# achraf-15/neural_image_compression

Measured on AMD Instinct MI355X. Metric: images/sec (256x256 RGB, batch 32) fwd+bwd, higher is better.
Workload: dtype f32; 1 GPU; cfg2: JointAutoregressiveHierarchical(M=192,K=1) fwd+rd_loss(lambda=0.01)+bwd+Adam, 32x3x256x256 per GPU, fp32; global_batch=32, parallelism=dp1, step=eager (autograd)

## Files before the change

include/lic.h:

```cpp
#ifndef LIC_H
#define LIC_H

#include <stddef.h>
#include <stdint.h>

#ifdef __cplusplus
extern "C" {
#endif

#define LIC_ABI_VERSION 4

typedef void* lic_stream_t;

enum lic_status {
  LIC_OK = 0,
  LIC_ERR_INVALID = -1,
  LIC_ERR_UNSUPPORTED = -2,
  LIC_ERR_LAUNCH = -3,
  LIC_ERR_WORKSPACE = -4
};

enum lic_epilogue {
  LIC_EPI_NONE = 0,
  LIC_EPI_LEAKY = 1,
// ... 413 lines not shown
} lic_adam_job;
int64_t lic_adam_plan(lic_adam_job* jobs, int32_t njobs);
int lic_adam_run(const lic_adam_job* jobs_device, int32_t njobs, int64_t total_blocks, const float* const* grads_host,
                 double lr, double beta1, double beta2, double eps, double weight_decay, double bias_correction1,
                 double bias_correction2, lic_stream_t stream);

int lic_grad_norm_partial(const lic_adam_job* jobs_device, int32_t njobs, int64_t total_blocks,
                          const float* const* grads_host, double* partials, lic_stream_t stream);
int lic_grad_norm_finish(const double* partials, int64_t nparts, double max_norm, int32_t count_skip, float* clip_state,
                         lic_stream_t stream);
int lic_adam_run_scaled(const lic_adam_job* jobs_device, int32_t njobs, int64_t total_blocks,
                        const float* const* grads_host, double lr, double beta1, double beta2, double eps,
                        double weight_decay, double bias_correction1, double bias_correction2, const float* clip_state,
                        int32_t skip_nonfinite, lic_stream_t stream);

int lic_adam_run_ema(const lic_adam_job* jobs_device, int32_t njobs, int64_t total_blocks,
                     const float* const* grads_host, double lr, double beta1, double beta2, double eps,
                     double weight_decay, double bias_correction1, double bias_correction2, float* const* ema_device,
                     double ema_weight, const float* clip_state, int32_t skip_nonfinite, lic_stream_t stream);
int lic_swap_run(const lic_adam_job* jobs_device, int32_t njobs, int64_t total_blocks, float* const* ema_device,
                 lic_stream_t stream);

enum { LIC_REDUCE_SLABS = 0, LIC_REDUCE_COLUMNS = 1 };
enum { LIC_REDUCE_EPI_NONE = 0, LIC_REDUCE_EPI_REPARAM = 1 };
#define LIC_REDUCE_MAX_JOBS 32
typedef struct lic_reduce_job {
  const float* src;
  float* dst;
  const float* param;
  int64_t sm, smr, sn, snr, stap;
  int32_t kind, epilogue;
  int32_t splitk, ntaps, Cm, Cn, Mvalid, Nvalid, mdiv, ndiv;
  float scale, bound;
  int32_t block0, nblocks;
} lic_reduce_job;
int lic_wgrad_bf16_partial(const lic_wgrad_desc* d, void* workspace, size_t workspace_bytes, lic_reduce_job* job,
                           lic_stream_t stream);
int lic_colsum_bf16_partial(const void* in, int64_t ld, int64_t P, int32_t C, float scale, float* out, void* workspace,
                            size_t workspace_bytes, lic_reduce_job* job, lic_stream_t stream);
int lic_colsum2_bf16_partial(const void* in_a, const void* in_b, int64_t ld, int64_t P, int32_t C, float scale,
                             float* out_a, float* out_b, void* workspace, size_t workspace_bytes, lic_reduce_job* jobs2,
                             lic_stream_t stream);
int lic_leaky_bwd_colsum_bf16(const void* y, const void* dy, void* dx, int64_t P, int32_t C, float slope, float* out,
                              void* workspace, size_t workspace_bytes, lic_reduce_job* job, lic_stream_t stream);
int lic_reduce_batch(const lic_reduce_job* jobs, int32_t njobs, lic_stream_t stream);

int lic_head_convt_bf16_supported(int32_t Cin, int32_t Cout, int32_t kh, int32_t kw, int32_t stride, int32_t pad,
                                  int32_t out_pad);
int lic_head_convt_bf16(const void* x, const void* w_packed, const float* bias, float* out, int32_t B, int32_t Hi,
                        int32_t Wi, int32_t Cin, lic_stream_t stream);
int lic_stem_conv_bf16(const float* x, const void* w_packed, const float* bias, void* y, int32_t B, int32_t H, int32_t W,
                       int32_t Cout, lic_stream_t stream);

typedef struct lic_plan lic_plan;
int lic_plan_create(void* hip_graph, lic_plan** out);
int lic_plan_info(const lic_plan* plan, int64_t* info);
int lic_plan_replay(lic_plan* plan, lic_stream_t main, const lic_stream_t* sides, int32_t n_sides);
int lic_plan_tune(lic_plan* plan, lic_stream_t main, const lic_stream_t* sides, int32_t n_sides, double* result);
int lic_plan_dag(const lic_plan* plan, int64_t cap_ops, int64_t cap_edges, int64_t* sizes, int32_t* pred_ptr,
                 int32_t* pred_idx, int32_t* kind, int32_t* flags, double* us);
int lic_plan_commands(lic_plan* plan, int32_t n_sides, int64_t cap, int64_t* n_cmds, int32_t* cmds);
int lic_plan_sched_host(int64_t n_ops, const int32_t* pred_ptr, const int32_t* pred_idx, const double* us,
                        const int32_t* flags, int32_t mode, int32_t ns, double wide_min_us, int32_t n_sides,
                        int64_t cap, int64_t* n_cmds, int32_t* cmds, int64_t* info);
void lic_plan_destroy(lic_plan* plan);
const char* lic_plan_last_error(void);

int lic_version(void);
int lic_last_hip_error(void);
const char* lic_arch(void);

#ifdef __cplusplus
}
#endif
#endif
```

neural_image_compression_amd/_lib.py:

```python
from __future__ import annotations

import ctypes as C
import os

_HERE = os.path.dirname(os.path.abspath(__file__))
LIB_PATH = os.path.join(_HERE, "liblic_hip.so")

EPI_NONE, EPI_LEAKY, EPI_MUL_LEAKY_MASK, EPI_GDN, EPI_IGDN, EPI_GDN_BWD, EPI_IGDN_BWD, EPI_CONV_GDN, EPI_CONV_IGDN = range(9)
FE_NPARAM = 43

_vp, _i32, _i64, _f32, _sz = C.c_void_p, C.c_int32, C.c_int64, C.c_float, C.c_size_t


class IgemmDesc(C.Structure):
    _fields_ = [("in_", _vp), ("w", _vp), ("bias", _vp), ("out", _vp), ("out2", _vp), ("aux", _vp),
                ("aux2", _vp), ("aux3", _vp), ("res", _vp),
                ("in_ld", _i64), ("out_ld", _i64), ("out2_ld", _i64), ("aux_ld", _i64),
                ("aux2_ld", _i64), ("aux3_ld", _i64), ("res_ld", _i64),
                ("B", _i32), ("Hi", _i32), ("Wi", _i32), ("Cin", _i32),
                ("Ho", _i32), ("Wo", _i32), ("Cout", _i32),
                ("kh", _i32), ("kw", _i32), ("stride", _i32), ("pad", _i32),
                ("transposed", _i32), ("prologue", _i32), ("epilogue", _i32),
                ("tap_mask", C.c_uint32), ("slope", _f32), ("workspace", _vp), ("workspace_bytes", _sz),
                ("out3", _vp), ("out3_ld", _i64),
# ... 171 lines not shown
    "lic_gdn_fwd": (C.c_int, [_vp, _vp, _vp, _vp, _vp, _vp, _i64, _i32, _i32, _vp]),
    "lic_gdn_bwd_partial_rows": (_i64, [_i64]),
    "lic_gdn_bwd": (C.c_int, [_vp, _vp, _vp, _vp, _vp, _vp, _vp, _vp, _i64, _i32, _i32, _vp]),
    "lic_factorized_cdf_tables": (C.c_int, [_vp, _i32, _i32, _i32, _vp, _vp]),
    "lic_gmm_cdf_tables": (C.c_int, [_vp, _i64, _i32, _i32, _i32, _vp, _vp, _vp]),
    "lic_rans_decode_step": (C.c_int, [_vp] * 8 + [_i32] * 4 + [_vp, _vp, _i64, _vp]),
    "lic_rans_encode_pick": (C.c_int, [_vp] * 4 + [_i32, _i64, _i32, _i32] + [_vp] * 4),
    "lic_rans_encode": (C.c_int, [_vp] * 3 + [_i64, _i32, _i64, _vp, _i64, _vp, _vp, _vp]),
    "lic_rans_decode_step_groups": (C.c_int, [_vp] * 8 + [_i32] * 5 + [_vp, _vp, _i64, _vp]),
    "lic_rans_encode_groups": (C.c_int, [_vp] * 3 + [_i64, _i32, _i32, _i64, _vp, _i64, _vp, _i64, _vp, _vp]),
    "lic_rans_encode_pick_ragged": (C.c_int, [_vp] * 3 + [_i64, _vp, _i32, _vp, _vp, _i32, _i32] + [_vp] * 4),
    "lic_rans_encode_ragged": (C.c_int, [_vp] * 3 + [_i64, _vp, _vp, _i32, _i32, _i64, _i32, _vp, _i64, _vp, _i64,
                                         _vp, _vp]),
    "lic_ctx_gather": (C.c_int, [_vp] + [_i64] * 4 + [_i32] * 4 + [_vp, _i32, _i32, _vp, _i64, _vp, _vp, _i32, _vp, _i64,
                                 _i32, _vp]),
    "lic_ctx_gather_ragged": (C.c_int, [_vp, _i64, _i64, _vp, _i32, _i32, _vp, _i32, _vp, _vp, _i64, _vp, _vp, _i64, _i32,
                                        _vp, _i64, _i32, _vp]),
    "lic_rans_decode_step_ragged": (C.c_int, [_vp] * 9 + [_i32, _i32, _i64, _i32, _i32, _vp, _vp, _vp, _vp, _i64, _vp]),
    "lic_ctx_gather_layers": (C.c_int, [_vp] + [_i64] * 4 + [_i32] * 3 + [_vp, _i32, _i32, _vp, _i64, _vp, _i32,
                                        C.POINTER(CtxLayer), _i32, _i32, _vp]),
    "lic_rans_decode_step_layers": (C.c_int, [_vp] * 6 + [C.POINTER(RansLayer)] + [_i32] * 5 + [_vp, _vp, _i64, _i64,
                                                                                                 _vp]),
    "lic_ctx_gather_layers_ragged": (C.c_int, [_vp, _i64, _i64, _vp, _i32, _vp, _i32, _vp, _vp, _i64, _vp, _i64, _i32,
                                               C.POINTER(CtxLayer), _i32, _i32, _vp]),
    "lic_rans_decode_step_layers_ragged": (C.c_int, [_vp] * 6 + [C.POINTER(RansLayer), _i32, _vp, _i32, _i32, _i64,
                                                                 _i32, _vp, _vp, _vp, _vp, _i64, _i64, _vp]),
    "lic_rans_z_pick": (C.c_int, [_vp, _i32, _i32, _i32, _vp, _i64, _vp, _vp, _vp, _vp]),
    "lic_rans_z_decode_path": (C.c_int, [_i32, _i32]),
    "lic_rans_z_decode": (C.c_int, [_vp] * 7 + [_i32] * 5 + [_vp, _vp, _vp, _i64, _i32, _vp]),
    "lic_msssim_workspace_bytes": (_sz, [_i32, _i32, _i32, _i32]),
    "lic_msssim": (C.c_int, [_vp, _vp, _i32, _i32, _i32, _i32, _i64, _i64, _i64, _i64, _f32, _vp, _vp, _vp, _sz,
                             _vp]),
    "lic_msssim_bwd_workspace_bytes": (_sz, [_i32, _i32, _i32, _i32]),
    "lic_msssim_bwd": (C.c_int, [_vp, _vp, _i32, _i32, _i32, _i32, _i64, _i64, _i64, _i64, _f32, _vp, _vp, _sz, _vp,
                                 _vp, _vp, _sz, _vp]),
    "lic_u8_to_f32": (C.c_int, [_vp, _vp, _i64, _vp]),
    "lic_window_u8_to_f32": (C.c_int, [_vp, _vp, _i32, _i32, _i32, _i32, _i32, _vp, _vp]),
    "lic_window_f32": (C.c_int, [_vp, _i64, _i64, _i64, _i64] + [_i32] * 9 + [_vp, _vp]),
    "lic_resample_u8_to_f32": (C.c_int, [_vp, _vp, _i32, _i32, _i32, _i32, _vp, _vp]),
    "lic_tensor_stats_workspace_bytes": (_sz, []),
    "lic_tensor_stats": (C.c_int, [_vp, _i64, _i32, _f32, _f32, _vp, _vp, _vp, _sz, _vp]),
    "lic_prep_plan": (_i64, [C.POINTER(PrepJob), _i32]),
    "lic_prep_run": (C.c_int, [_vp, _i32, _i64, _vp]),
    "lic_adam_plan": (_i64, [C.POINTER(AdamJob), _i32]),
    "lic_adam_run": (C.c_int, [_vp, _i32, _i64, _vp] + [C.c_double] * 7 + [_vp]),
    "lic_grad_norm_partial": (C.c_int, [_vp, _i32, _i64, _vp, _vp, _vp]),
    "lic_grad_norm_finish": (C.c_int, [_vp, _i64, C.c_double, _i32, _vp, _vp]),
    "lic_adam_run_scaled": (C.c_int, [_vp, _i32, _i64, _vp] + [C.c_double] * 7 + [_vp, _i32, _vp]),
    "lic_adam_run_ema": (C.c_int, [_vp, _i32, _i64, _vp] + [C.c_double] * 7 + [_vp, C.c_double, _vp, _i32, _vp]),
    "lic_swap_run": (C.c_int, [_vp, _i32, _i64, _vp, _vp]),
    "lic_head_convt_bf16_supported": (C.c_int, [_i32] * 7),
    "lic_head_convt_bf16": (C.c_int, [_vp, _vp, _vp, _vp, _i32, _i32, _i32, _i32, _vp]),
    "lic_stem_conv_bf16": (C.c_int, [_vp, _vp, _vp, _vp, _i32, _i32, _i32, _i32, _vp]),
    "lic_plan_create": (C.c_int, [_vp, C.POINTER(C.c_void_p)]),
    "lic_plan_info": (C.c_int, [_vp, C.POINTER(C.c_int64)]),
    "lic_plan_replay": (C.c_int, [_vp, _vp, C.POINTER(C.c_void_p), _i32]),
    "lic_plan_tune": (C.c_int, [_vp, _vp, C.POINTER(C.c_void_p), _i32, C.POINTER(C.c_double)]),
    "lic_plan_dag": (C.c_int, [_vp, _i64, _i64, C.POINTER(C.c_int64), _vp, _vp, _vp, _vp, _vp]),
    "lic_plan_commands": (C.c_int, [_vp, _i32, _i64, C.POINTER(C.c_int64), _vp]),
    "lic_plan_sched_host": (C.c_int, [_i64, _vp, _vp, _vp, _vp, _i32, _i32, C.c_double, _i32, _i64,
                                      C.POINTER(C.c_int64), _vp, _vp]),
    "lic_plan_destroy": (None, [_vp]),
    "lic_plan_last_error": (C.c_char_p, []),
    "lic_version": (C.c_int, []),
    "lic_last_hip_error": (C.c_int, []),
    "lic_arch": (C.c_char_p, []),
}

_lib = None


class LicError(RuntimeError):
    pass


def load():
    global _lib
    if _lib is None:
        if not os.path.exists(LIB_PATH):
            raise LicError(
                f"{LIB_PATH} not found: the HIP extension is not built. Run "
                "`python -c 'import __graft_entry__ as g; g.build()'` (or make -C "
                "neural_image_compression_amd/csrc). There is no CPU fallback.")
        lib = C.CDLL(LIB_PATH)
        for name, (res, args) in SIGNATURES.items():
            fn = getattr(lib, name)
            fn.restype = res
            fn.argtypes = args
        _lib = lib
    return _lib


_STATUS = {-1: "LIC_ERR_INVALID", -2: "LIC_ERR_UNSUPPORTED", -3: "LIC_ERR_LAUNCH", -4: "LIC_ERR_WORKSPACE"}


def check(rc: int, what: str):
    if rc != 0:
        extra = f" (hipError {load().lic_last_hip_error()})" if rc == -3 else ""
        raise LicError(f"{what} failed: {_STATUS.get(rc, rc)}{extra}")
```

neural_image_compression_amd/functional.py:

```python
from __future__ import annotations

import ctypes as C
from typing import Optional, Tuple

import torch

from . import _lib as L
from .reductions import can_defer, defer, flush_point, flush_reductions

PEDESTAL = float(2.0 ** -36)
LIKELIHOOD_BOUND = 1e-9

PROFILE = None
PROFILE_MIN_FLOP = 0.0
FORCE_IGEMM = None
FORCE_WGRAD = None
KERNEL_TRACE = None
GRAD_VIEWS = {}
PREPARED = {}
AUX_STREAM = None
PLAN_RECORDING = False


_raw_stream = getattr(torch._C, "_cuda_getCurrentRawStream", None)


def _stream():
    if _raw_stream is not None:
        return C.c_void_p(_raw_stream(torch.cuda.current_device()))
    return C.c_void_p(torch.cuda.current_stream().cuda_stream)


def _ptr(t: Optional[torch.Tensor]):
    return None if t is None else C.c_void_p(t.data_ptr())


def _require_cuda(*ts):
    for t in ts:
        if t is not None and not t.is_cuda:
            raise L.LicError("neural_image_compression_amd runs on MI355X only: got a non-CUDA tensor "
                             "(there is no CPU fallback; the CPU oracle lives in oracle/ for tests)")
        if t is not None and t.device.index != torch.cuda.current_device():
            raise L.LicError(f"tensor on cuda:{t.device.index} but the current device is cuda:"
                             f"{torch.cuda.current_device()}: call torch.cuda.set_device(...) first (one process per GPU)")
        if t is not None and t.dtype != torch.float32:
            raise L.LicError(f"fp32 tensors expected, got {t.dtype}")


def _nhwc(t: torch.Tensor) -> torch.Tensor:
    return t.permute(0, 2, 3, 1).contiguous()


def _nchw_view(t_nhwc: torch.Tensor) -> torch.Tensor:
    return t_nhwc.permute(0, 3, 1, 2)


def _permute3(src, dst, n, s, d):
    L.check(L.load().lic_permute3(_ptr(src), _ptr(dst), n[0], n[1], n[2], s[0], s[1], s[2], d[0], d[1],
                                  d[2], _stream()), "lic_permute3")


def _pack(src: torch.Tensor, taps: int, K: int, N: int, s_tap: int, s_k: int, s_n: int) -> torch.Tensor:
    lib = L.load()
    out = torch.empty((lib.lic_packed_weight_floats(taps, K, N),), device=src.device, dtype=torch.float32)
    L.check(lib.lic_pack_weight(_ptr(src), _ptr(out), taps, K, N, s_tap, s_k, s_n, _stream()),
            "lic_pack_weight")
    return out


def _pack_dense(m: torch.Tensor) -> torch.Tensor:
    K, N = m.shape
    return _pack(m, 1, K, N, 0, N, 1)

# ... 410 lines not shown
                                          ctx.needs_input_grad[1], has_bias and ctx.needs_input_grad[2])
        return dx, dw, db, None, None, None, None


class _ImageConvGDNFn(torch.autograd.Function):

    @staticmethod
    def forward(ctx, x, weight, bias, beta, gamma, stride, pad, inverse, beta_bound, gamma_bound, pedestal, keep=True):
        _require_cuda(x, weight, bias, beta, gamma)
        xh = _nhwc(x)
        B = xh.shape[0]
        Cout = weight.shape[0]
        col, wp, Ho, Wo, Kp = _image_conv_columns(xh, weight, stride, pad)
        P = B * Ho * Wo
        beta_e, gT = _gdn_operands(beta, gamma, beta_bound, gamma_bound, pedestal)
        y = torch.empty((B, Ho, Wo, Cout), device=x.device, dtype=torch.float32)
        conv_out = torch.empty_like(y) if keep else None
        norm = torch.empty_like(y) if keep else None
        _igemm(col, wp, y, B=1, Hi=1, Wi=P, Cin=Kp, Ho=1, Wo=P, Cout=Cout, kh=1, kw=1, stride=1,
               pad=0, transposed=False, bias=bias, epilogue=L.EPI_CONV_IGDN if inverse else L.EPI_CONV_GDN,
               out2=norm, out3=conv_out, aux=gT, aux2=beta_e)
        ctx.save_for_backward(col, weight, conv_out, norm, beta, gamma)
        ctx.cfg = (stride, pad, tuple(xh.shape), inverse, beta_bound, gamma_bound, bias is not None, pedestal)
        return _nchw_view(y)

    @staticmethod
    def backward(ctx, gy):
        col, weight, conv_out, norm, beta, gamma = ctx.saved_tensors
        stride, pad, in_shape, inverse, beta_bound, gamma_bound, has_bias, pedestal = ctx.cfg
        need = ctx.needs_input_grad
        g_conv, dbeta, dgamma = _gdn_backward(conv_out, norm, beta, gamma, _nhwc(gy), inverse,
                                              beta_bound, gamma_bound, pedestal, True, need[3], need[4])
        dx, dw, db = _image_conv_backward(col, weight, g_conv, stride, pad, in_shape, need[0], need[1],
                                          has_bias and need[2])
        return dx, dw, db, dbeta, dgamma, None, None, None, None, None, None, None


class _ImageConvTFn(torch.autograd.Function):

    @staticmethod
    def forward(ctx, x, weight, bias, stride, pad, out_pad):
        _require_cuda(x, weight, bias)
        xh = _nhwc(x)
        B, Hi, Wi, Cin = xh.shape
        _, Cout, kh, kw = weight.shape
        Ho, Wo = conv_out_size(Hi, Wi, kh, stride, pad, True, out_pad)
        taps, Kp, P = kh * kw, _kpad(kh, kw, Cout), B * Hi * Wi
        lib = L.load()
        wpk = prepared(weight, "f32.head")
        if wpk is None:
            wp = torch.zeros((Cin, Kp), device=x.device, dtype=torch.float32)
            _permute3(weight.contiguous(), wp, (Cin, Cout, taps), (Cout * taps, taps, 1), (Kp, 1, Cout))
            wpk = _pack_dense(wp)
        col = torch.empty((P, Kp), device=x.device, dtype=torch.float32)
        _igemm(xh, wpk, col, B=1, Hi=1, Wi=P, Cin=Cin, Ho=1, Wo=P, Cout=Kp, kh=1, kw=1, stride=1, pad=0,
               transposed=False)
        out = torch.empty((B, Ho, Wo, Cout), device=x.device, dtype=torch.float32)
        L.check(lib.lic_col2im(_ptr(col), _ptr(bias), _ptr(out), B, Hi, Wi, Cout, Ho, Wo, kh, kw, stride,
                               pad, Kp, _stream()), "lic_col2im")
        ctx.save_for_backward(xh, weight)
        ctx.cfg = (stride, pad, (Ho, Wo), bias is not None)
        return _nchw_view(out)

    @staticmethod
    def backward(ctx, gy):
        xh, weight = ctx.saved_tensors
        stride, pad, (Ho, Wo), has_bias = ctx.cfg
        g = _nhwc(gy)
        B, Hi, Wi, Cin = xh.shape
        _, Cout, kh, kw = weight.shape
        taps, Kp, P = kh * kw, _kpad(kh, kw, Cout), B * Hi * Wi
        lib = L.load()
        dcol = torch.empty((P, Kp), device=g.device, dtype=torch.float32)
        L.check(lib.lic_im2col(_ptr(g), _ptr(dcol), B, Ho, Wo, Cout, Hi, Wi, kh, kw, stride, pad, Kp,
                               _stream()), "lic_im2col")
        dx = dw = db = None
        if ctx.needs_input_grad[0]:
            wpk = prepared(weight, "f32.head_dx")
            if wpk is None:
                wpT = torch.zeros((Kp, Cin), device=g.device, dtype=torch.float32)
                _permute3(weight.contiguous(), wpT, (taps, Cout, Cin), (1, taps, Cout * taps),
                          (Cout * Cin, Cin, 1))
                wpk = _pack_dense(wpT)
            dxh = torch.empty_like(xh)
            _igemm(dcol, wpk, dxh, B=1, Hi=1, Wi=P, Cin=Kp, Ho=1, Wo=P, Cout=Cin, kh=1, kw=1, stride=1,
                   pad=0, transposed=False)
            dx = _nchw_view(dxh)
        if ctx.needs_input_grad[1]:
            dw = grad_like(weight)
            tmp = torch.empty((Cin, Kp), device=g.device, dtype=torch.float32)
            _wgrad(xh, dcol, tmp, B=1, Hs=1, Ws=P, Cp=Cin, Hl=1, Wl=P, Cg=Kp, kh=1, kw=1, stride=1, pad=0,
                   g_is_row=True, dst_sm=1, dst_sn=Kp, dst_stap=0)
            _permute3(tmp, dw, (Cin, taps, Cout), (Kp, Cout, 1), (Cout * taps, 1, taps))
        if has_bias and ctx.needs_input_grad[2]:
            db = _colsum(g, B * Ho * Wo, Cout)
        return dx, dw, db, None, None, None


def image_conv2d(x, weight, bias, stride, padding, leaky=False, slope=0.01):
    return _ImageConvFn.apply(x, weight, bias, stride, padding, leaky, slope)


def image_conv_transpose2d(x, weight, bias, stride, padding, output_padding):
    return _ImageConvTFn.apply(x, weight, bias, stride, padding, output_padding)


class _LeakyFn(torch.autograd.Function):
    @staticmethod
    def forward(ctx, x, slope):
        _require_cuda(x)
        xc = x.contiguous()
        y = _leaky_bwd(xc, xc, slope)
        ctx.save_for_backward(y)
        ctx.slope = slope
        return y

    @staticmethod
    def backward(ctx, gy):
        (y,) = ctx.saved_tensors
        return _leaky_bwd(y, gy.contiguous(), ctx.slope), None


def leaky_relu(x, slope=0.01):
    return _LeakyFn.apply(x, slope)


class _GDNFn(torch.autograd.Function):
    @staticmethod
    def forward(ctx, x, beta, gamma, inverse, beta_bound, gamma_bound, pedestal, res, keep=True):
        _require_cuda(x, beta, gamma, res)
        lib = L.load()
        xh = _nhwc(x)
        B, H, W, Cc = xh.shape
        beta_e, gT = _gdn_operands(beta, gamma, beta_bound, gamma_bound, pedestal)
        out = torch.empty_like(xh)
        norm = torch.empty_like(xh) if keep else None
        resh = None if res is None else _nhwc(res)
        P = B * H * W
        if lib.lic_gdn_supported(Cc):
            _trace(lambda: f"gdn_kernel<{Cc // 64}, {int(inverse)}>")
            _timed(f"gdn_kernel<{Cc // 64}, 0>", 2 * P * Cc * Cc, 4 * 3 * P * Cc,
                   lambda: L.check(lib.lic_gdn_fwd(_ptr(xh), _ptr(gT), _ptr(beta_e), _ptr(resh), _ptr(out), _ptr(norm),
                                                   P, Cc, int(inverse), _stream()), "lic_gdn_fwd"))
        else:
            _igemm(xh, gT, out, B=1, Hi=1, Wi=P, Cin=Cc, Ho=1, Wo=P, Cout=Cc, kh=1, kw=1, stride=1, pad=0,
                   transposed=False, bias=beta_e, prologue=1, epilogue=L.EPI_IGDN if inverse else L.EPI_GDN,
                   out2=norm, aux=xh, res=resh)
        ctx.save_for_backward(xh, norm, beta, gamma)
        ctx.cfg = (inverse, beta_bound, gamma_bound, res is not None, pedestal)
# ... 749 lines not shown
```

neural_image_compression_amd/csrc/lic_gemm.hip:

```cpp
#include "lic_tile_map.h"
#include <stdio.h>
#include <stdlib.h>
#include <algorithm>
#include <type_traits>

thread_local int g_lic_last_hip_error = 0;

struct IgemmParams {
  const float* in;
  const float* w;
  const float* bias;
  float* out;
  float* out2;
  const float* aux;
  const float* aux2;
  const float* aux3;
  const float* res;
  float* out3;
  long in_ld, out_ld, out2_ld, aux_ld, aux2_ld, aux3_ld, res_ld, out3_ld;
  int B, Hi, Wi, Cin, Ho, Wo, Cout;
  int kw, stride, pad, transposed, prologue, epilogue;
  float slope;
  int vec;
  int vec_out;
// ... 1175 lines not shown
          for (int b = 0; b < TN; ++b)
            acc[a][b] = __builtin_amdgcn_mfma_f32_32x32x2f32(af[a][t], bf[b][t], acc[a][b], 0, 0, 0);
    } else {
#pragma unroll
      for (int a = 0; a < TM; ++a)
        if (a < m_live) {
#pragma unroll
          for (int b = 0; b < TN; ++b)
            if (b < n_live) {
#pragma unroll
              for (int t = 0; t < 8; ++t)
                acc[a][b] = __builtin_amdgcn_mfma_f32_32x32x2f32(af[a][t], bf[b][t], acc[a][b], 0, 0, 0);
            }
        }
    }
  };

  if (nloc > 0) {
    load_chunk(c_begin);
    store_chunk(0);
    __syncthreads();
    load_chunk(c_begin + 1);
    int c = 0;
    for (; c + 1 < nloc; c += 2) {
      store_chunk(1);
      load_chunk(c_begin + c + 2);
      compute(0);
      __syncthreads();
      store_chunk(0);
      load_chunk(c_begin + c + 3);
      compute(1);
      __syncthreads();
    }
    if (c < nloc) {
      compute(0);
      __syncthreads();
    }
  }
  float* slab = p.slabs + ((long)split * p.ntaps + tap) * p.row.C * p.col.C;
#pragma unroll
  for (int a = 0; a < TM; ++a)
#pragma unroll
    for (int q = 0; q < 16; ++q) {
      const int m = m0 + wm0 + a * 32 + (q & 3) + 8 * (q >> 2) + 4 * lh;
      if (m >= p.row.C) continue;
#pragma unroll
      for (int b = 0; b < TN; ++b) {
        const int n = n0 + wn0 + b * 32 + li;
        if (n < p.col.C) slab[(long)m * p.col.C + n] = acc[a][b][q];
      }
    }
}

template <int TM, int TN, bool SQB = false, bool FULL = true>
__global__ __launch_bounds__(256, (TM * TN >= 6 ? 2 : 1)) void wgrad_glds_kernel(const WgradParams p) {
  constexpr int BMt = 64 * TM, BNt = 64 * TN, NS = TM + TN;
  constexpr int WM = BMt / 2, WN = BNt / 2;
  __shared__ __attribute__((aligned(16))) float smem[2][NS][WG_BK * 64];
  const int tid = threadIdx.x, lane = tid & 63;
  const int wave = __builtin_amdgcn_readfirstlane(tid >> 6);
  const int wm0 = (wave >> 1) * WM, wn0 = (wave & 1) * WN;
  const int li = lane & 31, lh = lane >> 5;
  const WgradTile wt = wgrad_tile(p, xcd_contiguous(blockIdx.x, gridDim.x), BMt, BNt);
  const int m0 = wt.m0, n0 = wt.n0, tap = wt.tap, split = wt.split;
  const int c_begin = wt.c_begin, c_end = wt.c_end, nloc = c_end - c_begin;

  f32x16 acc[TM][TN];
#pragma unroll
  for (int a = 0; a < TM; ++a)
#pragma unroll
    for (int b = 0; b < TN; ++b)
#pragma unroll
      for (int q = 0; q < 16; ++q) acc[a][b][q] = 0.0f;

  const int kr = tid >> 4, c16 = (tid & 15) * 4;
  constexpr unsigned WG_OOB = 0x80000000u, WG_GBIAS = 0x40000000u;
  const unsigned row_ld4 = (unsigned)p.row.ld * 4u, col_ld4 = (unsigned)p.col.ld * 4u;
  const unsigned row_lin = (unsigned)kr * row_ld4 + (unsigned)c16 * 4u;
  const unsigned col_lin = (unsigned)kr * col_ld4 + (unsigned)c16 * 4u;
  const bool row_g = p.row.gathered != 0, col_g = p.col.gathered != 0;
  const unsigned g_ld4 = row_g ? row_ld4 : col_ld4;
  const unsigned HWl = (unsigned)(p.Hl * p.Wl);
  const int tap_h = wt.r - p.pad, tap_w = wt.s - p.pad;
  bool row_live[TM], col_live[TN];
#pragma unroll
  for (int j = 0; j < TM; ++j) row_live[j] = FULL || m0 + c16 + 64 * j < p.row.C;
#pragma unroll
  for (int j = 0; j < TN; ++j) col_live[j] = FULL || n0 + c16 + 64 * j < p.col.C;
  const float* const row_base = p.row.ptr + m0;
  const float* const col_base = p.col.ptr + n0;
  auto issue = [&](int c, int buf) {
    const int cc = c < c_end ? c : c_end - 1;
    const int pk0 = cc * WG_BK;
    const int b0 = fdiv(pk0, p.dHW);
    const int rem0 = pk0 - b0 * p.Hs * p.Ws;
    const int hs0 = fdiv(rem0, p.dW), ws0 = rem0 - hs0 * p.Ws;
    const long g0 = ((long)b0 * p.Hl + (hs0 * p.stride + tap_h)) * p.Wl + (ws0 * p.stride + tap_w);
    const unsigned pk = (unsigned)pk0 + (unsigned)kr;
    const int pix = pk < (unsigned)p.Ps ? (int)pk : 0;
    const int b = fdiv(pix, p.dHW);
    const int rem = pix - b * p.Hs * p.Ws;
    const int hs = fdiv(rem, p.dW), ws = rem - hs * p.Ws;
    const int hl = hs * p.stride + tap_h, wl = ws * p.stride + tap_w;
    const bool gok = pk < (unsigned)p.Ps && (unsigned)hl < (unsigned)p.Hl && (unsigned)wl < (unsigned)p.Wl;
    const unsigned dpix = (unsigned)b * HWl + (unsigned)hl * (unsigned)p.Wl + (unsigned)wl - (unsigned)g0;
    const unsigned gokm = (unsigned)(-(int)gok);
    const unsigned g_off = ((dpix * g_ld4 + (WG_GBIAS + (unsigned)c16 * 4u)) & gokm) | (~gokm & WG_OOB);
    const long left = p.Ps - pk0;
    const unsigned lin_rec = (unsigned)(left < WG_BK ? left : WG_BK);
    auto rsrc = [&](const float* base, long ld, unsigned ld4, bool gathered) {
      const long px = gathered ? g0 : (long)pk0;
      const float* b_ = base + (px * ld - (gathered ? (long)(WG_GBIAS / 4) : 0L));
      return __builtin_amdgcn_make_buffer_rsrc(const_cast<float*>(b_), 0, gathered ? (int)WG_OOB : (int)(lin_rec * ld4),
                                               0x00020000);
    };
    const __amdgpu_buffer_rsrc_t rs_row = rsrc(row_base, p.row.ld, row_ld4, row_g);
    const __amdgpu_buffer_rsrc_t rs_col = rsrc(col_base, p.col.ld, col_ld4, col_g);
    const unsigned row_off = row_g ? g_off : row_lin, col_off = col_g ? g_off : col_lin;
#pragma unroll
    for (int j = 0; j < TM; ++j)
      __builtin_amdgcn_raw_ptr_buffer_load_lds(rs_row, (lic_lptr_t)&smem[buf][j][wave * 256], 16,
                                               (int)(row_live[j] ? row_off : WG_OOB), 256 * j, 0, 0);
#pragma unroll
    for (int j = 0; j < TN; ++j)
      __builtin_amdgcn_raw_ptr_buffer_load_lds(rs_col, (lic_lptr_t)&smem[buf][TM + j][wave * 256], 16,
                                               (int)(col_live[j] ? col_off : WG_OOB), 256 * j, 0, 0);
  };
  auto compute = [&](int buf) {
    float af[TM][8], bf[TN][8];
#pragma unroll
    for (int a = 0; a < TM; ++a) {
      const int ch = wm0 + a * 32;
#pragma unroll
      for (int t = 0; t < 8; ++t) af[a][t] = smem[buf][ch >> 6][(lh * 8 + t) * 64 + (ch & 63) + li];
    }
#pragma unroll
    for (int b = 0; b < TN; ++b) {
      const int ch = wn0 + b * 32;
#pragma unroll
      for (int t = 0; t < 8; ++t) {
        const float v = smem[buf][TM + (ch >> 6)][(lh * 8 + t) * 64 + (ch & 63) + li];
        bf[b][t] = SQB ? v * v : v;
      }
    }
#pragma unroll
    for (int t = 0; t < 8; ++t)
#pragma unroll
      for (int a = 0; a < TM; ++a)
#pragma unroll
        for (int b = 0; b < TN; ++b)
          acc[a][b] = __builtin_amdgcn_mfma_f32_32x32x2f32(af[a][t], bf[b][t], acc[a][b], 0, 0, 0);
  };

  if (nloc > 0) {
    issue(c_begin, 0);
    int c = 0;
    for (; c + 1 < nloc; c += 2) {
      __syncthreads();
      issue(c_begin + c + 1, 1);
      compute(0);
      __builtin_amdgcn_sched_barrier(0);
      __syncthreads();
      issue(c_begin + c + 2, 0);
      compute(1);
      __builtin_amdgcn_sched_barrier(0);
    }
    __syncthreads();
    if (c < nloc) compute(0);
  }
  float* slab = p.slabs + ((long)split * p.ntaps + tap) * p.row.C * p.col.C;
#pragma unroll
  for (int a = 0; a < TM; ++a)
#pragma unroll
    for (int q = 0; q < 16; ++q) {
      const int m = m0 + wm0 + a * 32 + (q & 3) + 8 * (q >> 2) + 4 * lh;
      if (!FULL && m >= p.row.C) continue;
#pragma unroll
      for (int b = 0; b < TN; ++b) {
        const int n = n0 + wn0 + b * 32 + li;
        if (FULL || n < p.col.C) slab[(long)m * p.col.C + n] = acc[a][b][q];
      }
    }
}

__global__ __launch_bounds__(256) void wgrad_reduce_kernel(const float* slabs, float* dst, int splitk,
                                                           int ntaps, int Cm, int Cn, long sm, long sn,
                                                           long stap, float scale) {
  const long total = (long)ntaps * Cm * Cn;
  for (long i = (long)blockIdx.x * 256 + threadIdx.x; i < total; i += (long)gridDim.x * 256) {
    float a8[8] = {0.f, 0.f, 0.f, 0.f, 0.f, 0.f, 0.f, 0.f};
    int z = 0;
    for (; z + 8 <= splitk; z += 8) {
#pragma unroll
      for (int k = 0; k < 8; ++k) a8[k] += slabs[(long)(z + k) * total + i];
    }
    for (; z < splitk; ++z) a8[0] += slabs[(long)z * total + i];
    const float acc = ((a8[0] + a8[1]) + (a8[2] + a8[3])) + ((a8[4] + a8[5]) + (a8[6] + a8[7]));
    const int n = (int)(i % Cn);
    const long t2 = i / Cn;
    const int m = (int)(t2 % Cm);
    const int tap = (int)(t2 / Cm);
    dst[m * sm + n * sn + tap * stap] = acc * scale;
  }
}

long lic_pick_splits(long base, long slots, long max_sk) {
  long best = 1;
  double best_eff = 0.0;
  if (max_sk > 512) max_sk = 512;
  if (max_sk < 1) max_sk = 1;
  for (long r = 1; r <= 4; ++r) {
    long sk = (r * slots) / base;
    if (sk < 1) continue;
    if (sk > max_sk) sk = max_sk;
    const long wgs = base * sk;
    const double eff = (double)wgs / ((double)((wgs + slots - 1) / slots) * (double)slots);
    if (eff > best_eff + 0.03) {
      best = sk;
      best_eff = eff;
    }
    if (eff >= 0.9 || sk == max_sk) break;
// ... 157 lines not shown
```

Measured before the change: 1496 images/s.

## Fuse RGB head transposed-conv GEMM and col2im into one direct kernel

Adds a dedicated fp32 MFMA kernel for the final 5x5 stride-2 transposed conv to 3 channels. Each tile computes the per-pixel column products into LDS with halo and immediately scatters and adds them into the output image, so the large intermediate column buffer is never written to or read back from global memory. The kernel is persistent and software-pipelines input and weight loads. It recomputes the halo columns in each tile and only covers specific channel counts, falling back to the old GEMM plus col2im path otherwise.

```diff
diff --git a/include/lic.h b/include/lic.h
--- a/include/lic.h
+++ b/include/lic.h
@@ -489,6 +489,11 @@
 int lic_stem_conv_bf16(const float* x, const void* w_packed, const float* bias, void* y, int32_t B, int32_t H, int32_t W,
                        int32_t Cout, lic_stream_t stream);
 
+int lic_head_convt_f32_supported(int32_t Cin, int32_t Cout, int32_t kh, int32_t kw, int32_t stride, int32_t pad,
+                                 int32_t out_pad);
+int lic_head_convt_f32(const float* x, const float* w_packed, const float* bias, float* out, int32_t B, int32_t Hi, int32_t Wi,
+                       int32_t Cin, int32_t grid_cap, lic_stream_t stream);
+
 typedef struct lic_plan lic_plan;
 int lic_plan_create(void* hip_graph, lic_plan** out);
 int lic_plan_info(const lic_plan* plan, int64_t* info);
diff --git a/neural_image_compression_amd/_lib.py b/neural_image_compression_amd/_lib.py
--- a/neural_image_compression_amd/_lib.py
+++ b/neural_image_compression_amd/_lib.py
@@ -247,6 +247,8 @@
     "lic_head_convt_bf16_supported": (C.c_int, [_i32] * 7),
     "lic_head_convt_bf16": (C.c_int, [_vp, _vp, _vp, _vp, _i32, _i32, _i32, _i32, _vp]),
     "lic_stem_conv_bf16": (C.c_int, [_vp, _vp, _vp, _vp, _i32, _i32, _i32, _i32, _vp]),
+    "lic_head_convt_f32_supported": (C.c_int, [_i32] * 7),
+    "lic_head_convt_f32": (C.c_int, [_vp, _vp, _vp, _vp, _i32, _i32, _i32, _i32, _i32, _vp]),
     "lic_plan_create": (C.c_int, [_vp, C.POINTER(C.c_void_p)]),
     "lic_plan_info": (C.c_int, [_vp, C.POINTER(C.c_int64)]),
     "lic_plan_replay": (C.c_int, [_vp, _vp, C.POINTER(C.c_void_p), _i32]),
diff --git a/neural_image_compression_amd/csrc/lic_rgb.hip b/neural_image_compression_amd/csrc/lic_rgb.hip
--- /dev/null
+++ b/neural_image_compression_amd/csrc/lic_rgb.hip
@@ -0,0 +1,188 @@
+#include "lic_common.h"
+
+namespace {
+
+__device__ __forceinline__ void rg_lds_barrier() { asm volatile("s_waitcnt lgkmcnt(0)\n\ts_barrier" ::: "memory"); }
+
+constexpr int HF_TH = 12, HF_TW = 16;
+constexpr int HF_HR = HF_TH + 2, HF_HC = HF_TW + 2;
+constexpr int HF_HP = HF_HR * HF_HC;
+constexpr int HF_MT = (HF_HP + 31) / 32;
+constexpr int HF_LD = 84;
+constexpr int HF_THREADS = 64 * HF_MT;
+
+struct HeadFwdParams {
+  const float* x;
+  const float* w;
+  const float* bias;
+  float* out;
+  int B, Hi, Wi, tiles_x, tiles_y;
+  long ntiles;
+};
+
+template <int NC>
+__global__ __launch_bounds__(HF_THREADS, 2) void head_convt_f32_kernel(const HeadFwdParams p) {
+  constexpr int C = 16 * NC;
+  constexpr int WTS = NC * 3 * 512;
+  __shared__ __attribute__((aligned(16))) float smem[WTS + HF_MT * 32 * HF_LD];
+  float* wts = smem;
+  float* col = smem + WTS;
+  const int tid = threadIdx.x, lane = tid & 63, li = lane & 31, lh = lane >> 5;
+  const int wave = __builtin_amdgcn_readfirstlane(tid >> 6);
+  for (int v = tid; v < WTS / 4; v += HF_THREADS) {
+    const int blk = v >> 6, c = blk / 6, r = blk - 6 * c;
+    *reinterpret_cast<f32x4*>(wts + 4 * v) = *reinterpret_cast<const f32x4*>(p.w + ((long)(c * 8 + r) * 64 + (v & 63)) * 4);
+  }
+  float bs[3] = {0.f, 0.f, 0.f};
+  if (p.bias)
+#pragma unroll
+    for (int c = 0; c < 3; ++c) bs[c] = p.bias[c];
+  const int Ho = 2 * p.Hi, Wo = 2 * p.Wi;
+  const int ntiles = (int)p.ntiles;
+  const float* wl = wts + lane * 4;
+  const int hp = 32 * wave + li;
+  const int hr = hp / HF_HC, hc = hp - hr * HF_HC;
+  auto row_of = [&](int tile) {
+    const int tx = tile % p.tiles_x, rest = tile / p.tiles_x;
+    const int ty = rest % p.tiles_y, b = rest / p.tiles_y;
+    const int iy = min(max(ty * HF_TH - 1 + hr, 0), p.Hi - 1), ix = min(max(tx * HF_TW - 1 + hc, 0), p.Wi - 1);
+    return p.x + (((long)b * p.Hi + iy) * p.Wi + ix) * C + 8 * lh;
+  };
+  f32x4 a[3][2];
+  f32x4 bw[2][3][2];
+  const float* xrow = p.x;
+  auto load_a = [&](int c) {
+    a[c % 3][0] = *reinterpret_cast<const f32x4*>(xrow + 16 * c);
+    a[c % 3][1] = *reinterpret_cast<const f32x4*>(xrow + 16 * c + 4);
+  };
+  auto load_b = [&](int c) {
+#pragma unroll
+    for (int nt = 0; nt < 3; ++nt)
+#pragma unroll
+      for (int q = 0; q < 2; ++q) bw[c & 1][nt][q] = *reinterpret_cast<const f32x4*>(wl + ((c * 3 + nt) * 2 + q) * 256);
+  };
+  int tile = blockIdx.x;
+  if (tile < ntiles) {
+    xrow = row_of(tile);
+    load_a(0);
+    load_a(1);
+  }
+  rg_lds_barrier();
+
+  for (; tile < ntiles; tile += gridDim.x) {
+    const int tx = tile % p.tiles_x, rest = tile / p.tiles_x;
+    const int ty = rest % p.tiles_y, b = rest / p.tiles_y;
+    const int y0 = ty * HF_TH, x0 = tx * HF_TW;
+    f32x16 acc[3];
+#pragma unroll
+    for (int nt = 0; nt < 3; ++nt)
+#pragma unroll
+      for (int r = 0; r < 16; ++r) acc[nt][r] = 0.0f;
+    load_b(0);
+#pragma unroll
+    for (int c = 0; c < NC; ++c) {
+      if (c + 2 < NC) load_a(c + 2);
+      if (c + 1 < NC) load_b(c + 1);
+      __builtin_amdgcn_sched_barrier(0);
+#pragma unroll
+      for (int t = 0; t < 8; ++t)
+#pragma unroll
+        for (int nt = 0; nt < 3; ++nt)
+          acc[nt] = __builtin_amdgcn_mfma_f32_32x32x2f32(a[c % 3][t >> 2][t & 3], bw[c & 1][nt][t >> 2][t & 3], acc[nt], 0, 0, 0);
+    }
+    {
+      float* dst = col + (32 * wave + 4 * lh) * HF_LD + li;
+#pragma unroll
+      for (int nt = 0; nt < 3; ++nt)
+        if (32 * nt + li < 80)
+#pragma unroll
+          for (int r = 0; r < 16; ++r) dst[((r & 3) + 8 * (r >> 2)) * HF_LD + 32 * nt] = acc[nt][r] + 0.0f;
+    }
+    if (tile + (int)gridDim.x < ntiles) {
+      xrow = row_of(tile + gridDim.x);
+      load_a(0);
+      load_a(1);
+    }
+    rg_lds_barrier();
+    for (int o = tid; o < 4 * HF_TH * HF_TW; o += HF_THREADS) {
+      const int oyl = o / (2 * HF_TW), oxl = o - oyl * (2 * HF_TW);
+      const int oy = 2 * y0 + oyl, ox = 2 * x0 + oxl;
+      if (oy >= Ho || ox >= Wo) continue;
+      const int qy = oyl >> 1, py = oyl & 1, qx = oxl >> 1, px = oxl & 1;
+      float o0 = bs[0], o1 = bs[1], o2 = bs[2];
+#pragma unroll
+      for (int aa = 0; aa < 3; ++aa) {
+        const int ky = py + 2 * aa, iy = y0 + qy + 1 - aa;
+        if (ky > 4 || iy < 0 || iy >= p.Hi) continue;
+#pragma unroll
+        for (int bb = 0; bb < 3; ++bb) {
+          const int kx = px + 2 * bb, ix = x0 + qx + 1 - bb;
+          if (kx > 4 || ix < 0 || ix >= p.Wi) continue;
+          const float* c3 = col + ((qy + 2 - aa) * HF_HC + (qx + 2 - bb)) * HF_LD + 3 * (5 * ky + kx);
+          o0 += c3[0];
+          o1 += c3[1];
+          o2 += c3[2];
+        }
+      }
+      float* dst = p.out + (((long)b * Ho + oy) * Wo + ox) * 3;
+      dst[0] = o0;
+      dst[1] = o1;
+      dst[2] = o2;
+    }
+    rg_lds_barrier();
+  }
+}
+
+bool rg_al16(const void* q) { return (reinterpret_cast<uintptr_t>(q) & 15) == 0; }
+
+template <int NC>
+int head_fwd_launch(const HeadFwdParams& p, int grid_cap, hipStream_t s) {
+  static const int slots = [] {
+    int per_cu = 0, cus = 0, devid = 0;
+    if (hipOccupancyMaxActiveBlocksPerMultiprocessor(&per_cu, (const void*)head_convt_f32_kernel<NC>, HF_THREADS, 0) != hipSuccess ||
+        per_cu < 1)
+      per_cu = 1;
+    if (hipGetDevice(&devid) != hipSuccess ||
+        hipDeviceGetAttribute(&cus, hipDeviceAttributeMultiprocessorCount, devid) != hipSuccess || cus < 1)
+      cus = 256;
+    return per_cu * cus;
+  }();
+  long grid = p.ntiles < slots ? p.ntiles : slots;
+  if (grid_cap > 0 && grid > grid_cap) grid = grid_cap;
+  hipLaunchKernelGGL((head_convt_f32_kernel<NC>), dim3((unsigned)grid), dim3(HF_THREADS), 0, s, p);
+  return lic_check_launch();
+}
+
+bool rg_geometry(int Cin, int Cout, int kh, int kw, int stride, int pad, int out_pad) {
+  return (Cin == 64 || Cin == 128 || Cin == 192) && Cout == 3 && kh == 5 && kw == 5 && stride == 2 && pad == 2 && out_pad == 1;
+}
+
+}
+
+LIC_EXPORT int lic_head_convt_f32_supported(int32_t Cin, int32_t Cout, int32_t kh, int32_t kw, int32_t stride, int32_t pad,
+                                            int32_t out_pad) {
+  return rg_geometry(Cin, Cout, kh, kw, stride, pad, out_pad) ? 1 : 0;
+}
+
+LIC_EXPORT int lic_head_convt_f32(const float* x, const float* w_packed, const float* bias, float* out, int32_t B, int32_t Hi,
+                                  int32_t Wi, int32_t Cin, int32_t grid_cap, lic_stream_t stream) {
+  if (!x || !w_packed || !out || B <= 0 || Hi <= 0 || Wi <= 0 || grid_cap < 0) return LIC_ERR_INVALID;
+  if (!(Cin == 64 || Cin == 128 || Cin == 192)) return LIC_ERR_UNSUPPORTED;
+  if (!rg_al16(x) || !rg_al16(w_packed) || (reinterpret_cast<uintptr_t>(out) & 3)) return LIC_ERR_INVALID;
+  if ((long)B * Hi * Wi * Cin > 0x7FFFFFFFFFL || (long)B * Hi * Wi >= 0x7FFFFFFFL) return LIC_ERR_UNSUPPORTED;
+  HeadFwdParams p;
+  p.x = x;
+  p.w = w_packed;
+  p.bias = bias;
+  p.out = out;
+  p.B = B;
+  p.Hi = Hi;
+  p.Wi = Wi;
+  p.tiles_x = (Wi + HF_TW - 1) / HF_TW;
+  p.tiles_y = (Hi + HF_TH - 1) / HF_TH;
+  p.ntiles = (long)B * p.tiles_x * p.tiles_y;
+  hipStream_t s = (hipStream_t)stream;
+  if (Cin == 64) return head_fwd_launch<4>(p, grid_cap, s);
+  if (Cin == 128) return head_fwd_launch<8>(p, grid_cap, s);
+  return head_fwd_launch<12>(p, grid_cap, s);
+}
diff --git a/neural_image_compression_amd/functional.py b/neural_image_compression_amd/functional.py
--- a/neural_image_compression_amd/functional.py
+++ b/neural_image_compression_amd/functional.py
@@ -19,6 +19,7 @@
 GRAD_VIEWS = {}
 PREPARED = {}
 AUX_STREAM = None
+RGB_DIRECT = True
 PLAN_RECORDING = False
 
 
@@ -535,12 +536,15 @@
             wp = torch.zeros((Cin, Kp), device=x.device, dtype=torch.float32)
             _permute3(weight.contiguous(), wp, (Cin, Cout, taps), (Cout * taps, taps, 1), (Kp, 1, Cout))
             wpk = _pack_dense(wp)
-        col = torch.empty((P, Kp), device=x.device, dtype=torch.float32)
-        _igemm(xh, wpk, col, B=1, Hi=1, Wi=P, Cin=Cin, Ho=1, Wo=P, Cout=Kp, kh=1, kw=1, stride=1, pad=0,
-               transposed=False)
         out = torch.empty((B, Ho, Wo, Cout), device=x.device, dtype=torch.float32)
-        L.check(lib.lic_col2im(_ptr(col), _ptr(bias), _ptr(out), B, Hi, Wi, Cout, Ho, Wo, kh, kw, stride,
-                               pad, Kp, _stream()), "lic_col2im")
+        if RGB_DIRECT and xh.numel() < 2 ** 31 and lib.lic_head_convt_f32_supported(Cin, Cout, kh, kw, stride, pad, out_pad):
+            _head_fwd_direct(xh, wpk, bias, out)
+        else:
+            col = torch.empty((P, Kp), device=x.device, dtype=torch.float32)
+            _igemm(xh, wpk, col, B=1, Hi=1, Wi=P, Cin=Cin, Ho=1, Wo=P, Cout=Kp, kh=1, kw=1, stride=1, pad=0,
+                   transposed=False)
+            L.check(lib.lic_col2im(_ptr(col), _ptr(bias), _ptr(out), B, Hi, Wi, Cout, Ho, Wo, kh, kw, stride,
+                                   pad, Kp, _stream()), "lic_col2im")
         ctx.save_for_backward(xh, weight)
         ctx.cfg = (stride, pad, (Ho, Wo), bias is not None)
         return _nchw_view(out)
@@ -578,6 +582,15 @@
         if has_bias and ctx.needs_input_grad[2]:
             db = _colsum(g, B * Ho * Wo, Cout)
         return dx, dw, db, None, None, None
+
+
+def _head_fwd_direct(xh, wpk, bias, out, grid_cap=0):
+    B, Hi, Wi, Cin = xh.shape
+    name = f"head_convt_f32_kernel<{Cin // 16}>"
+    _trace(name)
+    _timed(name, 2.0 * B * Hi * Wi * Cin * 75, 4 * (B * Hi * Wi * Cin + 12 * B * Hi * Wi),
+           lambda: L.check(L.load().lic_head_convt_f32(_ptr(xh), _ptr(wpk), _ptr(bias), _ptr(out), B, Hi, Wi, Cin, grid_cap,
+                                                       _stream()), "lic_head_convt_f32"))
 
 
 def image_conv2d(x, weight, bias, stride, padding, leaky=False, slope=0.01):
```

Measured after the change: 1501 images/s (median of 6 runs). Within noise of the previous version (+0.3%).

## Add triple-buffered LDS ring with split-half register pipelining to 3x3 wgrad kernel

Applied to the files above, without the earlier changes.

For the TM=3,TN=3 weight-gradient kernel, LDS staging goes from two buffers to a three-slot ring. Fragment reads are split into two halves using inline ds_read2st64_b32 with explicit lgkmcnt waits, so LDS reads of one half overlap the MFMAs of the other. The next global-to-LDS load is issued while compute is running. Branchy descriptor selection in issue is also replaced by mask arithmetic. This adds LDS footprint, which can lower occupancy, and depends on hand-written waitcnt ordering being correct.

```diff
diff --git a/neural_image_compression_amd/csrc/lic_gemm.hip b/neural_image_compression_amd/csrc/lic_gemm.hip
--- a/neural_image_compression_amd/csrc/lic_gemm.hip
+++ b/neural_image_compression_amd/csrc/lic_gemm.hip
@@ -1251,11 +1251,14 @@
     }
 }
 
+typedef float f32x2 __attribute__((ext_vector_type(2)));
+constexpr bool wgrad_ring(int TM, int TN) { return TM == 3 && TN == 3; }
 template <int TM, int TN, bool SQB = false, bool FULL = true>
 __global__ __launch_bounds__(256, (TM * TN >= 6 ? 2 : 1)) void wgrad_glds_kernel(const WgradParams p) {
   constexpr int BMt = 64 * TM, BNt = 64 * TN, NS = TM + TN;
   constexpr int WM = BMt / 2, WN = BNt / 2;
-  __shared__ __attribute__((aligned(16))) float smem[2][NS][WG_BK * 64];
+  constexpr bool RING = wgrad_ring(TM, TN);
+  __shared__ __attribute__((aligned(16))) float smem[RING ? 3 : 2][NS][WG_BK * 64];
   const int tid = threadIdx.x, lane = tid & 63;
   const int wave = __builtin_amdgcn_readfirstlane(tid >> 6);
   const int wm0 = (wave >> 1) * WM, wn0 = (wave & 1) * WN;
@@ -1278,6 +1281,7 @@
   const unsigned row_lin = (unsigned)kr * row_ld4 + (unsigned)c16 * 4u;
   const unsigned col_lin = (unsigned)kr * col_ld4 + (unsigned)c16 * 4u;
   const bool row_g = p.row.gathered != 0, col_g = p.col.gathered != 0;
+  const long row_gm = -(long)row_g, col_gm = -(long)col_g;
   const unsigned g_ld4 = row_g ? row_ld4 : col_ld4;
   const unsigned HWl = (unsigned)(p.Hl * p.Wl);
   const int tap_h = wt.r - p.pad, tap_w = wt.s - p.pad;
@@ -1307,15 +1311,16 @@
     const unsigned g_off = ((dpix * g_ld4 + (WG_GBIAS + (unsigned)c16 * 4u)) & gokm) | (~gokm & WG_OOB);
     const long left = p.Ps - pk0;
     const unsigned lin_rec = (unsigned)(left < WG_BK ? left : WG_BK);
-    auto rsrc = [&](const float* base, long ld, unsigned ld4, bool gathered) {
-      const long px = gathered ? g0 : (long)pk0;
-      const float* b_ = base + (px * ld - (gathered ? (long)(WG_GBIAS / 4) : 0L));
-      return __builtin_amdgcn_make_buffer_rsrc(const_cast<float*>(b_), 0, gathered ? (int)WG_OOB : (int)(lin_rec * ld4),
-                                               0x00020000);
+    auto rsrc = [&](const float* base, long ld, unsigned ld4, long gm) {
+      const long px = (g0 & gm) | ((long)pk0 & ~gm);
+      const float* b_ = base + (px * ld - ((long)(WG_GBIAS / 4) & gm));
+      return __builtin_amdgcn_make_buffer_rsrc(const_cast<float*>(b_), 0,
+                                               (int)((WG_OOB & (unsigned)gm) | (lin_rec * ld4 & ~(unsigned)gm)), 0x00020000);
     };
-    const __amdgpu_buffer_rsrc_t rs_row = rsrc(row_base, p.row.ld, row_ld4, row_g);
-    const __amdgpu_buffer_rsrc_t rs_col = rsrc(col_base, p.col.ld, col_ld4, col_g);
-    const unsigned row_off = row_g ? g_off : row_lin, col_off = col_g ? g_off : col_lin;
+    const __amdgpu_buffer_rsrc_t rs_row = rsrc(row_base, p.row.ld, row_ld4, row_gm);
+    const __amdgpu_buffer_rsrc_t rs_col = rsrc(col_base, p.col.ld, col_ld4, col_gm);
+    const unsigned row_off = (g_off & (unsigned)row_gm) | (row_lin & ~(unsigned)row_gm);
+    const unsigned col_off = (g_off & (unsigned)col_gm) | (col_lin & ~(unsigned)col_gm);
 #pragma unroll
     for (int j = 0; j < TM; ++j)
       __builtin_amdgcn_raw_ptr_buffer_load_lds(rs_row, (lic_lptr_t)&smem[buf][j][wave * 256], 16,
@@ -1325,47 +1330,147 @@
       __builtin_amdgcn_raw_ptr_buffer_load_lds(rs_col, (lic_lptr_t)&smem[buf][TM + j][wave * 256], 16,
                                                (int)(col_live[j] ? col_off : WG_OOB), 256 * j, 0, 0);
   };
-  auto compute = [&](int buf) {
-    float af[TM][8], bf[TN][8];
+  if constexpr (RING) {
+    constexpr int BUF_UNITS = NS * 16;
+    static_assert(2 * BUF_UNITS + 7 <= 255, "ds_read2st64_b32 offsets are 8 bits");
+    const unsigned lds0 = (unsigned)(size_t)(__attribute__((address_space(3))) void*)&smem[0][0][0];
+    unsigned fa_addr[TM], fb_addr[TN];
 #pragma unroll
     for (int a = 0; a < TM; ++a) {
       const int ch = wm0 + a * 32;
-#pragma unroll
-      for (int t = 0; t < 8; ++t) af[a][t] = smem[buf][ch >> 6][(lh * 8 + t) * 64 + (ch & 63) + li];
+      fa_addr[a] = lds0 + 4u * (unsigned)((ch >> 6) * (WG_BK * 64) + lh * 8 * 64 + (ch & 63) + li);
     }
 #pragma unroll
     for (int b = 0; b < TN; ++b) {
       const int ch = wn0 + b * 32;
-#pragma unroll
-      for (int t = 0; t < 8; ++t) {
-        const float v = smem[buf][TM + (ch >> 6)][(lh * 8 + t) * 64 + (ch & 63) + li];
-        bf[b][t] = SQB ? v * v : v;
-      }
-    }
-#pragma unroll
-    for (int t = 0; t < 8; ++t)
+      fb_addr[b] = lds0 + 4u * (unsigned)((TM + (ch >> 6)) * (WG_BK * 64) + lh * 8 * 64 + (ch & 63) + li);
+    }
+    auto read_h = [&](auto bufc, auto hc, f32x2 (&af)[TM][2], f32x2 (&bf)[TN][2]) {
+      constexpr int buf = decltype(bufc)::value, h = decltype(hc)::value;
+      constexpr int o = buf * BUF_UNITS + 4 * h;
 #pragma unroll
       for (int a = 0; a < TM; ++a)
 #pragma unroll
-        for (int b = 0; b < TN; ++b)
-          acc[a][b] = __builtin_amdgcn_mfma_f32_32x32x2f32(af[a][t], bf[b][t], acc[a][b], 0, 0, 0);
-  };
-
-  if (nloc > 0) {
-    issue(c_begin, 0);
-    int c = 0;
-    for (; c + 1 < nloc; c += 2) {
+        for (int q = 0; q < 2; ++q) {
+          const unsigned ad = fa_addr[a];
+          asm volatile("ds_read2st64_b32 %0, %1 offset0:%2 offset1:%3"
+                       : "=v"(af[a][q])
+                       : "v"(ad), "i"(o + 2 * q), "i"(o + 2 * q + 1));
+        }
+#pragma unroll
+      for (int b = 0; b < TN; ++b)
+#pragma unroll
+        for (int q = 0; q < 2; ++q) {
+          const unsigned ad = fb_addr[b];
+          asm volatile("ds_read2st64_b32 %0, %1 offset0:%2 offset1:%3"
+                       : "=v"(bf[b][q])
+                       : "v"(ad), "i"(o + 2 * q), "i"(o + 2 * q + 1));
+        }
+    };
+    auto arrive = [&](auto newerc, f32x2 (&af)[TM][2], f32x2 (&bf)[TN][2], bool square) {
+      asm volatile("s_waitcnt lgkmcnt(%0)" ::"i"(decltype(newerc)::value) : "memory");
+#pragma unroll
+      for (int a = 0; a < TM; ++a)
+#pragma unroll
+        for (int q = 0; q < 2; ++q) asm volatile("" : "+v"(af[a][q]));
+#pragma unroll
+      for (int b = 0; b < TN; ++b)
+#pragma unroll
+        for (int q = 0; q < 2; ++q) {
+          asm volatile("" : "+v"(bf[b][q]));
+          if (SQB && square) bf[b][q] = bf[b][q] * bf[b][q];
+        }
+    };
+    auto mfma_h = [&](const f32x2 (&af)[TM][2], const f32x2 (&bf)[TN][2]) {
+#pragma unroll
+      for (int t = 0; t < 4; ++t)
+#pragma unroll
+        for (int a = 0; a < TM; ++a)
+#pragma unroll
+          for (int b = 0; b < TN; ++b)
+            acc[a][b] = __builtin_amdgcn_mfma_f32_32x32x2f32(af[a][t >> 1][t & 1], bf[b][t >> 1][t & 1], acc[a][b], 0,
+                                                              0, 0);
+    };
+    if (nloc > 0) {
+      using I0 = std::integral_constant<int, 0>;
+      using I1 = std::integral_constant<int, 1>;
+      using I2 = std::integral_constant<int, 2>;
+      using NF = std::integral_constant<int, 2 * NS>;
+      static_assert(2 * NS <= 15, "lgkmcnt is 4 bits");
+      f32x2 a0[TM][2], b0[TN][2], a1[TM][2], b1[TN][2];
+      issue(c_begin, 0);
+      issue(c_begin + 1, 1);
+      asm volatile("s_waitcnt vmcnt(%0)\n\ts_barrier" ::"i"(NS) : "memory");
+      read_h(I0{}, I0{}, a0, b0);
+      int cn = c_begin + 2;
+      auto step = [&](auto cur, auto nxt, auto fill) {
+        asm volatile("s_waitcnt vmcnt(0)\n\ts_barrier" ::: "memory");
+        read_h(cur, I1{}, a1, b1);
+        arrive(NF{}, a0, b0, true);
+        __builtin_amdgcn_sched_barrier(0);
+        issue(cn++, decltype(fill)::value);
+        mfma_h(a0, b0);
+        __builtin_amdgcn_sched_barrier(0);
+        read_h(nxt, I0{}, a0, b0);
+        arrive(NF{}, a1, b1, true);
+        __builtin_amdgcn_sched_barrier(0);
+        mfma_h(a1, b1);
+        __builtin_amdgcn_sched_barrier(0);
+      };
+      int c = 0;
+      for (; c + 2 < nloc; c += 3) {
+        step(I0{}, I1{}, I2{});
+        step(I1{}, I2{}, I0{});
+        step(I2{}, I0{}, I1{});
+      }
+      if (c < nloc) step(I0{}, I1{}, I2{});
+      if (c + 1 < nloc) step(I1{}, I2{}, I0{});
+      arrive(I0{}, a0, b0, false);
       __syncthreads();
-      issue(c_begin + c + 1, 1);
-      compute(0);
-      __builtin_amdgcn_sched_barrier(0);
+    }
+  } else {
+    auto compute = [&](int buf) {
+      float af[TM][8], bf[TN][8];
+#pragma unroll
+      for (int a = 0; a < TM; ++a) {
+        const int ch = wm0 + a * 32;
+#pragma unroll
+        for (int t = 0; t < 8; ++t) af[a][t] = smem[buf][ch >> 6][(lh * 8 + t) * 64 + (ch & 63) + li];
+      }
+#pragma unroll
+      for (int b = 0; b < TN; ++b) {
+        const int ch = wn0 + b * 32;
+#pragma unroll
+        for (int t = 0; t < 8; ++t) {
+          const float v = smem[buf][TM + (ch >> 6)][(lh * 8 + t) * 64 + (ch & 63) + li];
+          bf[b][t] = SQB ? v * v : v;
+        }
+      }
+#pragma unroll
+      for (int t = 0; t < 8; ++t)
+#pragma unroll
+        for (int a = 0; a < TM; ++a)
+#pragma unroll
+          for (int b = 0; b < TN; ++b)
+            acc[a][b] = __builtin_amdgcn_mfma_f32_32x32x2f32(af[a][t], bf[b][t], acc[a][b], 0, 0, 0);
+    };
+
+    if (nloc > 0) {
+      issue(c_begin, 0);
+      int c = 0;
+      for (; c + 1 < nloc; c += 2) {
+        __syncthreads();
+        issue(c_begin + c + 1, 1);
+        compute(0);
+        __builtin_amdgcn_sched_barrier(0);
+        __syncthreads();
+        issue(c_begin + c + 2, 0);
+        compute(1);
+        __builtin_amdgcn_sched_barrier(0);
+      }
       __syncthreads();
-      issue(c_begin + c + 2, 0);
-      compute(1);
-      __builtin_amdgcn_sched_barrier(0);
-    }
-    __syncthreads();
-    if (c < nloc) compute(0);
+      if (c < nloc) compute(0);
+    }
   }
   float* slab = p.slabs + ((long)split * p.ntaps + tap) * p.row.C * p.col.C;
 #pragma unroll
```

New measurement: 1497 images/s before, 1479 images/s after. -1.2%, worse.
